# mrmod/h264decode

Hardware: AMD Instinct MI355X
Metric: 1080p Main CABAC frames/sec (higher is better)
Workload: dtype u8; 1 GPU; 1920x1080 Main CABAC IPPP GOP-30, 256 independent streams per GPU (32 distinct, each used 8 times), QP 28, 1 slice/frame, 1 ref; parallelism=streams sharded, no collective

## Files before the change

### h264decode_amd/csrc/k_entropy.hip

```cpp
#include <hip/hip_runtime.h>
#include "mi_kernels.h"

#ifndef MI_ENT_ISLICE_PRIO
#define MI_ENT_ISLICE_PRIO 0
#endif
#ifndef MI_ENT_MINWAVES
#define MI_ENT_MINWAVES 6
#endif
#ifndef MI_ENT_B
#define MI_ENT_B 0
#endif
#ifndef MI_ENT_FMO
#define MI_ENT_FMO MI_ENT_B
#endif
#ifndef MI_ENT_CABAC
#define MI_ENT_CABAC 0
#endif
#if MI_ENT_CABAC
#define ENT_CABAC(e) 1
#define IF_CAVLC(x) 0
#else
#define ENT_CABAC(e) ((e).cabac)
#define IF_CAVLC(x) (x)
#endif
// ... 26 lines not shown
    int8_t ipm[4];
    uint8_t nnz[8];
    int8_t ref[2][2];
    int16_t mv[NL][4][2];
    uint8_t mvd[NL][4][2];
};
#define TOP_DW (static_cast<int>(sizeof(TopInfo) / 4))
static_assert(sizeof(TopInfo) == (MI_ENT_B ? 72 : 48), "TopInfo layout");

struct Shared {
    uint8_t ctx[464];
#if !MI_ENT_CABAC
    uint8_t posmap[4][64];
#endif
    int16_t coef[MI_COEF_PER_MB];
    MbRec rec;
    TopInfo nb[4];
    int8_t ipm_c[32];
    uint8_t nnz_c[32];
    uint8_t nnzc_c[2][12];
    int8_t ref_c[NL][32];
    int8_t refi_c[NL][32];
    alignas(4) int16_t mv_c[NL][32][2];
    alignas(2) uint8_t mvd_c[NL][32][2];
    uint16_t parts[16];
    int8_t refs8[2][4];
    int8_t sub_type[4];
    uint8_t cur_cbf_dc, pad[3];
    int16_t ref_slot[NL][MI_MAX_REFS];
    uint32_t skip_tmpl[32];
    uint32_t role[64];
#if !MI_ENT_CABAC
    uint16_t vlc[MI_VLC_N];
#endif
    uint8_t coded[64];
#if MI_ENT_B
    uint32_t col[20];
    alignas(4) int16_t dmv[2][16][2];
    int8_t dref[2][4];
    int16_t dsf[MI_MAX_REFS];
#endif
};
#define GI(bx, by) (((by) + 1) * 6 + (bx) + 1)
enum { NB_LEFT = 0, NB_TL = 1, NB_TOP = 2 };

struct Ent {
    int lane;
    Shared *s;
    TopInfo *top;
    uint32_t pre_top;
// ... 498 lines not shown
        const int idx = st - 1, bx = (idx & 1) + 2 * ((idx >> 2) & 1), by = ((idx >> 1) & 1) + 2 * (idx >> 3);
        return static_cast<uint32_t>(GI(bx - 1, by)) | static_cast<uint32_t>(GI(bx, by - 1)) << 6 | static_cast<uint32_t>(GI(bx, by)) << 12 |
               static_cast<uint32_t>((by * 4 + bx) * 4) << 18 | 1u << 26;
    }
    if (st <= 18) {
        const uint32_t c = st - 17;
        return (51u + c) | (54u + c) << 6 | (57u + c) << 12 | (MI_COEF_CDC / 4 + c) << 18 | 2u << 26;
    }
    if (st <= 26) {
        const int j = st - 19, c = j >> 2, bx = j & 1, by = (j >> 1) & 1, g = 32 + 9 * c;
        return static_cast<uint32_t>(g + (by + 1) * 3 + bx) | static_cast<uint32_t>(g + by * 3 + bx + 1) << 6 | static_cast<uint32_t>(g + (by + 1) * 3 + bx + 1) << 12 |
               static_cast<uint32_t>(MI_COEF_CAC / 4 + j * 4) << 18 | 3u << 26;
    }
    return 0;
}
FI void parse_residual_cabac(Ent &e, int cbp_luma, int cbp_chroma, int t8x8) {
    Shared *s = e.s;
    const int i16 = e.cur_type == MBT_I16x16;
    int nl = LANE;
    OPAQUE(nl);
    const uint32_t cd = s->coded[nl];
    uint32_t vnz = (cd == 1 || (cd == 2 && MB_IS_INTRA(e.cur_type))) ? 1u : 0u;
    const uint32_t spread = (cbp_luma & 1) | (cbp_luma & 2) << 3 | (cbp_luma & 4) << 6 | (cbp_luma & 8) << 9;
    uint32_t steps = static_cast<uint32_t>(i16) | (spread * (t8x8 ? 1u : 15u)) << 1;
    if (cbp_chroma) steps |= 3u << 17;
    if (cbp_chroma & 2) steps |= 0xFFu << 19;
    const uint32_t cats = 0u | (t8x8 ? 5u : (i16 ? 1u : 2u)) << 4 | 3u << 8 | 4u << 12;
    while (steps) {
        const int step = __builtin_ctz(steps);
        steps &= steps - 1;
        const uint32_t d = RDL(e.v_step, step);
        const int cat = static_cast<int>((cats >> ((d >> 24) & 12u)) & 15);
        const int own = static_cast<int>((d >> 12) & 63);
        const int dst = cat == 5 ? (step - 1) * 16 : static_cast<int>((d >> 18) & 255) * 4;
        const int inc = static_cast<int>(RDL(vnz, d) + 2 * RDL(vnz, d >> 6));
        slide_window(e);
        if (cabac_residual(e, s->coef + dst, cat, inc)) {
            const uint64_t m = (cat == 5 ? 0xC3ull : 1ull) << own;
            asm("v_cndmask_b32_e64 %0, %0, 1, %1" : "+v"(vnz) : "s"(m));
        }
    }
    const uint64_t nzm = __builtin_amdgcn_ballot_w64(vnz != 0);
    const uint32_t lo = static_cast<uint32_t>(nzm);
    const uint32_t nzmask = ((lo >> GI(0, 0)) & 15) | ((lo >> GI(0, 1)) & 15) << 4 | ((lo >> GI(0, 2)) & 15) << 8 | ((lo >> GI(0, 3)) & 15) << 12;
    s->rec.nzmask = static_cast<uint16_t>(nzmask);
    s->cur_cbf_dc = static_cast<uint8_t>((nzm >> 56) & 7);
    int l = LANE;
    OPAQUE(l);
    const int bit = static_cast<int>(vnz);
    if (l < 30) {
        const int gx = l % 6 - 1, gy = l / 6 - 1;
        if (gx >= 0 && gx < 4 && gy >= 0) s->nnz_c[l] = static_cast<uint8_t>(bit);
    } else if (l >= 32 && l < 50) {
        const int i = l - 32, g = i % 9, gx = g % 3 - 1, gy = g / 3 - 1;
        if (gx >= 0 && gy >= 0) s->nnzc_c[i / 9][g] = static_cast<uint8_t>(bit);
    }
}

#if !MI_ENT_CABAC
FI void parse_residual_cavlc(Ent &e, int cbp_luma, int cbp_chroma, int t8x8) {
    Shared *s = e.s;
    const int i16 = e.cur_type == MBT_I16x16;
    int nzmask = 0, dc = 0;
    int nl = LANE;
    OPAQUE(nl);
    uint32_t vnn = nl < 30 ? s->nnz_c[nl] : ((nl >= 32 && nl < 56) ? (&s->nnzc_c[0][0])[nl - 32] : 0u);
    for (int step = 0; step < 27; step++) {
        int kind, bx = 0, by = 0, la = 0, lb = 0, own = 63, pmul = 1, padd = 0;
        int16_t *dst;
        if (step == 0) {
            if (!i16) continue;
            kind = 0;
            dst = s->coef + MI_COEF_I16DC;
            la = GI(-1, 0), lb = GI(0, -1);
        } else if (step <= 16) {
// ... 26 lines not shown
            la = 32 + 12 * c + (by + 1) * 3 + bx, lb = 32 + 12 * c + by * 3 + bx + 1, own = 32 + 12 * c + (by + 1) * 3 + bx + 1;
        }
        slide_window(e);
        const int nC = kind == 2 ? -1 : nc_of(static_cast<uint8_t>(RDL(vnn, la)), static_cast<uint8_t>(RDL(vnn, lb)));
        const int n = cavlc_residual(e, dst, kind, nC, pmul, padd);
        if (step == 0)
            dc |= n ? 1 : 0;
        else if (step <= 16) {
            vnn = nl == own ? static_cast<uint32_t>(n) : vnn;
            if (n) nzmask |= t8x8 ? (0x33 << ((by & 2) * 4 + (bx & 2))) : (1 << (by * 4 + bx));
        } else if (step <= 18)
            dc |= n ? 2 << (step - 17) : 0;
        else
            vnn = nl == own ? static_cast<uint32_t>(n) : vnn;
    }
    if (dc) s->cur_cbf_dc |= static_cast<uint8_t>(dc);
    s->rec.nzmask = static_cast<uint16_t>(nzmask);
    if (nl < 30) {
        const int gx = nl % 6 - 1, gy = nl / 6 - 1;
        if (gx >= 0 && gx < 4 && gy >= 0) s->nnz_c[nl] = static_cast<uint8_t>(vnn);
    } else if (nl >= 32 && nl < 56) {
        const int g = (nl - 32) % 12, gx = g % 3 - 1, gy = g / 3 - 1;
        if (g < 9 && gx >= 0 && gy >= 0) (&s->nnzc_c[0][0])[nl - 32] = static_cast<uint8_t>(vnn);
    }
}
#endif

FI int median3(int a, int b, int c) {
    int mn = a < b ? a : b, mx = a < b ? b : a;
    return c < mn ? mn : (c > mx ? mx : c);
}
FI void predict_mv(const Ent &e, const int L, int bx, int by, int w, int ref, int shape, int &px, int &py) {
    const Shared *s = e.s;
    int ia = GI(bx - 1, by), ib = GI(bx, by - 1), ic = GI(bx + w, by - 1);
    int ra = s->ref_c[L][ia], rb = s->ref_c[L][ib], rc = s->ref_c[L][ic];
    if (rc == -2) {
        ic = GI(bx - 1, by - 1);
        rc = s->ref_c[L][ic];
    }
// ... 56 lines not shown
        uint32_t off = NO_SRC, left = 0;
        if (gy < 0 && gx >= 0)
            off = NB_TOP * TB + static_cast<uint32_t>(offsetof(TopInfo, nnz)) + 4 + cpl * 2 + gx;
        else if (gx < 0 && gy >= 0)
            off = NB_LEFT * TB + static_cast<uint32_t>(offsetof(TopInfo, nnz)) + 4 + cpl * 2 + gy, left = 1;
        const uint32_t interior = gx >= 0 && gy >= 0;
        return off | interior << 12 | left << 14 | static_cast<uint32_t>(cpl * 12 + g) << 16;
    }
    if (l >= 50 && l < 56) {
        const uint32_t left = l < 53;
        return ((left ? NB_LEFT : NB_TOP) * TB + static_cast<uint32_t>(offsetof(TopInfo, cbf_dc))) | static_cast<uint32_t>((l - 50) % 3) << 9 | left << 14;
    }
    return NO_SRC;
}

FI void fill_caches(Ent &e) {
    Shared *s = e.s;
    const bool a_ok = (e.aw & 255) != 0, b_ok = (e.bw & 255) != 0;
    const int cip = e.cip;
    int l = LANE;
    OPAQUE(l);
    const uint32_t role = s->role[l], off = role & NO_SRC;
    const uint8_t *nbb = reinterpret_cast<const uint8_t *>(s->nb);
    int coded = 0;
    if (l < 30) {
        int8_t ipm = -2;
        uint8_t nnz = 0x80;
        const int k = static_cast<int>((role >> 9) & 3u);
        const bool has = off != NO_SRC && !((role >> 13) & 1u && e.mbx + 1 >= e.wmb);
        const TopInfo *n = reinterpret_cast<const TopInfo *>(nbb + (off != NO_SRC ? off : 0u));
        const bool n_ok = has && n->type != MBT_NONE;
        if (n_ok) {
            const int inter = MB_IS_INTER(n->type);
            if (!(cip && inter)) ipm = (n->type == MBT_I4x4 || n->type == MBT_I8x8) ? n->ipm[k] : static_cast<int8_t>(2);
            if ((role >> 11) & 1u) nnz = n->nnz[k];
        }
#pragma unroll
        for (int L = 0; L < NL; L++) {
            int8_t ref = -2, refi = -2;
            uint8_t mvdx = 0, mvdy = 0;
            int16_t mvx = 0, mvy = 0;
            if (n_ok) {
                if (MB_IS_INTER(n->type)) {
                    ref = refi = n->ref[L][k >> 1];
                    mvx = n->mv[L][k][0], mvy = n->mv[L][k][1];
                    mvdx = n->mvd[L][k][0], mvdy = n->mvd[L][k][1];
                    if (MI_ENT_B && ((n->dmask >> (k >> 1)) & 1)) refi = 0;
                } else
                    ref = refi = -1;
            }
            s->ref_c[L][l] = ref;
            s->refi_c[L][l] = refi;
            s->mv_c[L][l][0] = mvx, s->mv_c[L][l][1] = mvy;
            s->mvd_c[L][l][0] = mvdx, s->mvd_c[L][l][1] = mvdy;
        }
        if ((role >> 12) & 1u) {
            nnz = 0;
            ipm = -1;
        }
        coded = (nnz & 0x80) ? 2 : (nnz != 0);
        s->ipm_c[l] = ipm;
        e.v_ipm = ipm;
        s->nnz_c[l] = nnz;
    } else if (l >= 32 && l < 50) {
        const bool ok = off != NO_SRC && (((role >> 14) & 1u) ? a_ok : b_ok);
        const uint8_t v = ((role >> 12) & 1u) ? static_cast<uint8_t>(0) : (ok ? nbb[off != NO_SRC ? off : 0u] : static_cast<uint8_t>(0x80));
        coded = (v & 0x80) ? 2 : (v != 0);
        (&s->nnzc_c[0][0])[(role >> 16) & 31u] = v;
    } else if (l >= 50 && l < 56) {
        const bool ok = ((role >> 14) & 1u) ? a_ok : b_ok;
        coded = ok ? (nbb[off] >> ((role >> 9) & 3u)) & 1 : 2;
    } else if (l >= 56) {
        s->refs8[(l - 56) >> 2][l & 3] = -1;
        if (l < 60) s->sub_type[l - 56] = 0;
        if (l == 60) s->cur_cbf_dc = 0;
    }
    s->coded[l] = static_cast<uint8_t>(coded);
    LDS_SYNC();
}

#if MI_ENT_B
FI int min_positive(int a, int b) { return (a >= 0 && b >= 0) ? min(a, b) : max(a, b); }
FI int b_pair_modes(int k) { return static_cast<int>((0xFB7ED69A5ull >> (4 * k)) & 15); }
FI int b_sub_mode(int st) { return static_cast<int>((0x39FA5E4u >> (2 * st)) & 3); }
FI int b_sub_shape(int st) { return static_cast<int>((0x3F99900u >> (2 * st)) & 3); }
static_assert(((0x39FA5E4u >> 8) & 3) == 1 && ((0x39FA5E4u >> 24) & 3) == 3 && ((0x39FA5E4u >> 12) & 3) == 2 && ((0x3F99900u >> 8) & 3) == 1 && ((0x3F99900u >> 10) & 3) == 2,
              "Table 7-18 constants");

FI void direct_pred(Ent &e, int mask8, bool commit) {
    Shared *s = e.s;
    int l = LANE;
    OPAQUE(l);
    if (l < 20) s->col[l] = e.v_col;
// ... 171 lines not shown
        reinterpret_cast<uint32_t *>(e.top + e.mbx)[l] = nw;
        e.pre_top = top_load(e, e.mbx + 3, l);
    } else if (l >= 32) {
        const int k = l - 32;
        const uint32_t t = s->skip_tmpl[k];
        const uint32_t w = k == 0 ? (static_cast<uint32_t>(MBT_PSKIP) | e.qpw0) : (k == 1 ? e.qpw1 : ((k >= 12 && k < 28) ? mvw : t));
        const uint64_t mbi = e.mb_base + static_cast<uint64_t>(e.mby) * e.wmb + e.mbx;
        reinterpret_cast<uint32_t *>(e.mbrec + mbi)[k] = w;
    }
    LDS_SYNC();
}
#endif

FI void decode_mb(Ent &e, int skipped) {
    Shared *s = e.s;
    MbRec &r = s->rec;
    const int cabac = ENT_CABAC(e), islice = e.islice;
    int cbp_luma = 0, cbp_chroma = 0, t8x8 = 0, i16mode = 0, chroma_mode = 0, has_coef = 0;
    int type, raw = 0, nparts = 0;
    const Nb a{e.aw}, b{e.bw};
    r.nzmask = 0;
#if MI_ENT_B
    int no_sub8 = 1;
    e.direct8 = 0;
#endif
    if (skipped) {
#if MI_ENT_B
        type = MBT_BSKIP;
        e.cur_type = type;
        e.direct8 = 15;
        direct_pred(e, 15, true);
#else
        type = MBT_PSKIP;
        e.cur_type = type;
        int mvx = 0, mvy = 0;
        int ra = s->ref_c[0][GI(-1, 0)], rb = s->ref_c[0][GI(0, -1)];
        bool zero = ra == -2 || rb == -2 || (ra == 0 && s->mv_c[0][GI(-1, 0)][0] == 0 && s->mv_c[0][GI(-1, 0)][1] == 0) ||
                    (rb == 0 && s->mv_c[0][GI(0, -1)][0] == 0 && s->mv_c[0][GI(0, -1)][1] == 0);
        if (!zero) predict_mv(e, 0, 0, 0, 4, 0, 0, mvx, mvy);
        set_part(e, 0, 0, 0, 4, 4, 0, mvx, mvy, 0, 0);
        s->refs8[0][0] = s->refs8[0][1] = s->refs8[0][2] = s->refs8[0][3] = 0;
#endif
        e.prev_dqp_nz = 0;
    } else {
        MI_S(e, 3);
        int intra_prefix = 1;
        if (cabac) {
#if MI_ENT_B
            {
                intra_prefix = 0;
                const int inc = (a.ok() && a.type() != MBT_BSKIP && a.type() != MBT_BDIRECT) + (b.ok() && b.type() != MBT_BSKIP && b.type() != MBT_BDIRECT);
                if (!BIN_A(e, 27 + inc))
                    raw = 0;
                else if (!BIN_A(e, 27 + 3))
                    raw = 1 + BINI_A(e, 27 + 5);
                else {
                    int bits = BINI_A(e, 27 + 4) << 3;
                    bits |= BINI_A(e, 27 + 5) << 2;
                    bits |= BINI_A(e, 27 + 5) << 1;
// ... 57 lines not shown
        } else if (it == 25)
            type = MBT_IPCM;
        else {
            e.err = 20;
            type = MBT_I4x4;
        }
        e.cur_type = type;
        MI_S(e, 0);
        if (type == MBT_IPCM) {
            uint32_t pos = bitpos(e);
            if (cabac) pos -= static_cast<uint32_t>(RFL(e.avail));
            seek(e, (pos + 7) & ~7u);
            uint32_t *pcm = reinterpret_cast<uint32_t *>(s->coef);
            for (int i = 0; i < 96; i++) pcm[i] = (e.mono && i >= 64) ? 0x80808080u : __builtin_bswap32(get_bits(e, 32));
            if (cabac) cabac_start(e);
            for (int i = 0; i < 16; i++) {
                s->nnz_c[GI(i & 3, i >> 2)] = 16, s->ref_c[0][GI(i & 3, i >> 2)] = -1;
                if (MI_ENT_B) s->ref_c[NL - 1][GI(i & 3, i >> 2)] = -1;
            }
            for (int i = 0; i < 8; i++) s->nnzc_c[i >> 2][(((i >> 1) & 1) + 1) * 3 + (i & 1) + 1] = 16;
            s->cur_cbf_dc = 7;
            r.nzmask = 0xFFFF;
            cbp_luma = 15, cbp_chroma = 2;
            has_coef = 1;
            e.prev_dqp_nz = 0;
        } else {
            if (MB_IS_INTER(type)) {
#if MI_ENT_B
                if (type == MBT_BDIRECT) {
                    e.direct8 = 15;
                    direct_pred(e, 15, true);
                    no_sub8 = e.d8inf;
                } else {
                    int nref_parts;
                    if (raw <= 3) {
                        s->parts[0] = static_cast<uint16_t>(PART(0, 0, 4, 4, 0) | (raw << 11));
                        nparts = nref_parts = 1;
// ... 60 lines not shown
                        }
#pragma unroll
                    for (int L = 0; L < 2; L++)
                        for (int i = 0; i < nparts; i++) {
                            const int p = s->parts[i], md = p >> 11;
                            const int bx = p & 3, by = (p >> 2) & 3;
                            if (md == 0)
                                commit_direct(e, L, (by >> 1) * 2 + (bx >> 1));
                            else if ((md >> L) & 1)
                                read_mv(e, L, p);
                            else
                                set_part(e, L, bx, by, ((p >> 4) & 3) + 1, ((p >> 6) & 3) + 1, -1, 0, 0, 0, 0);
                        }
                }
#else
                int nref_parts;
                if (type == MBT_P16x16) {
                    s->parts[0] = PART(0, 0, 4, 4, 0);
                    nparts = nref_parts = 1;
                } else if (type == MBT_P16x8) {
                    s->parts[0] = PART(0, 0, 4, 2, 1), s->parts[1] = PART(0, 2, 4, 2, 2);
                    nparts = nref_parts = 2;
                } else if (type == MBT_P8x16) {
                    s->parts[0] = PART(0, 0, 2, 4, 3), s->parts[1] = PART(2, 0, 2, 4, 4);
                    nparts = nref_parts = 2;
                } else {
                    nref_parts = 4;
                    for (int i = 0; i < 4; i++) {
                        int st;
                        if (cabac)
// ... 14 lines not shown
                        bx = (i & 1) * 2, by = (i >> 1) * 2, w = 2, h = 2;
                    else {
                        const int p = s->parts[i];
                        bx = p & 3, by = (p >> 2) & 3, w = ((p >> 4) & 3) + 1, h = ((p >> 6) & 3) + 1;
                    }
                    read_ref_idx(e, 0, bx, by, w, h, raw != 4 ? e.nref : 1);
                }
                for (int i = 0; i < nparts; i++) read_mv(e, 0, s->parts[i]);
#endif
            } else {
                if (type == MBT_I4x4 && e.t8x8_mode) {
                    t8x8 = cabac ? BINI_T8(e, (a.ok() && a.t8x8()) + (b.ok() && b.t8x8())) : IF_CAVLC(static_cast<int>(get_bit(e)));
                    if (t8x8) type = MBT_I8x8, e.cur_type = type;
                }
                if (type == MBT_I4x4 || type == MBT_I8x8) {
                    const int n = type == MBT_I8x8 ? 4 : 16;
                    for (int i = 0; i < n; i++) {
                        int bx, by;
                        if (n == 4)
                            bx = (i & 1) * 2, by = (i >> 1) * 2;
                        else
                            bx = (i & 1) + 2 * ((i >> 2) & 1), by = ((i >> 1) & 1) + 2 * (i >> 3);
                        const int pa = static_cast<int>(RDL(e.v_ipm, GI(bx - 1, by))), pb = static_cast<int>(RDL(e.v_ipm, GI(bx, by - 1)));
                        const int pred = (pa < -1 || pb < -1) ? 2 : (pa < pb ? pa : pb);
                        int mode = pred;
                        if (cabac) {
                            if (!BIN_B(e, 68)) {
                                int rem = 0;
                                for (int k = 0; k < 3; k++) rem |= BINI_B(e, 69) << k;
                                mode = rem < pred ? rem : rem + 1;
// ... 9 lines not shown
                }
                if (e.mono)
                    chroma_mode = 0;
                else if (cabac) {
                    int inc = (a.ok() && MB_IS_INTRA(a.type()) && a.type() != MBT_IPCM && a.chroma_mode() != 0) +
                              (b.ok() && MB_IS_INTRA(b.type()) && b.type() != MBT_IPCM && b.chroma_mode() != 0);
                    chroma_mode = 0;
                    if (BIN_B(e, 64 + inc)) {
                        chroma_mode = 1;
                        while (chroma_mode < 3 && BIN_B(e, 67)) chroma_mode++;
                    }
                } else {
                    chroma_mode = IF_CAVLC(static_cast<int>(get_ue(e)));
                    if (chroma_mode > 3) e.err = 22, chroma_mode = 0;
                }
                if (LANE < 16) {
                    s->ref_c[0][GI(LANE & 3, LANE >> 2)] = -1;
                    if (MI_ENT_B) s->ref_c[NL - 1][GI(LANE & 3, LANE >> 2)] = -1;
                }
            }
            MI_S(e, MB_IS_INTER(type) ? 1 : 2);
            if (type != MBT_I16x16) {
                int cbp;
                if (cabac) {
                    const int cbp_a = a.ok() ? (a.type() == MBT_IPCM ? 0x2F : a.cbp()) : 0x0F;
                    const int cbp_b = b.ok() ? (b.type() == MBT_IPCM ? 0x2F : b.cbp()) : 0x0F;
                    cbp = 0;
                    for (int b8 = 0; b8 < 4; b8++) {
                        int ca = (b8 & 1) ? (cbp >> (b8 - 1)) & 1 : (cbp_a >> (b8 + 1)) & 1;
                        int cb = (b8 & 2) ? (cbp >> (b8 - 2)) & 1 : (cbp_b >> (b8 + 2)) & 1;
                        cbp |= BINI_B(e, 73 + (!ca) + 2 * (!cb)) << b8;
                    }
                    int ca = a.ok() && (a.type() == MBT_IPCM || (a.cbp() >> 4) != 0), cb = b.ok() && (b.type() == MBT_IPCM || (b.cbp() >> 4) != 0);
                    if (!e.mono && BIN_B(e, 77 + ca + 2 * cb)) {
// ... 26 lines not shown
                    while (BIN_A(e, 60 + ctx)) {
                        ctx = 2 + (ctx >> 1);
                        if (++val > 104) {
                            e.err = 2;
                            break;
                        }
                    }
                    dqp = (val & 1) ? (val + 1) >> 1 : -((val + 1) >> 1);
                } else
                    dqp = IF_CAVLC(get_se(e));
                if (dqp < -26 || dqp > 25) e.err = 24, dqp = 0;
                e.prev_dqp_nz = dqp != 0;
                if (dqp) set_qp(e, (e.qp + dqp + 52) % 52);
                MI_S(e, 2);
                MI_T(e, 1);
                MI_R0(e);
                if (cabac)
                    parse_residual_cabac(e, cbp_luma, cbp_chroma, t8x8);
                else
                    IF_CAVLC((parse_residual_cavlc(e, cbp_luma, cbp_chroma, t8x8), 0));
                MI_R(e, 3);
                MI_T(e, 2);
                has_coef = 1;
            } else
                e.prev_dqp_nz = 0;
        }
    }
    MI_T(e, 1);
    const int qp_store = type == MBT_IPCM ? 0 : e.qp;
    r.type = static_cast<uint8_t>(type);
    r.t8x8 = static_cast<uint8_t>(t8x8);
    r.qp = static_cast<uint8_t>(qp_store);
    r.qpc[0] = static_cast<uint8_t>(RDL(e.v_qpc, min(max(qp_store + e.cqp_off0, 0), 51)));
    r.qpc[1] = static_cast<uint8_t>(RDL(e.v_qpc, min(max(qp_store + e.cqp_off1, 0), 51)));
    r.cbp = static_cast<uint8_t>(cbp_luma | (cbp_chroma << 4));
    r.chroma_mode = static_cast<uint8_t>(chroma_mode);
    r.i16mode = static_cast<uint8_t>(i16mode);
    {
        const int cip = e.cip;
        int av = 0;
        if (MB_IS_INTRA(type)) {
            const int td = s->nb[NB_TL].type, tc = nb_ok(e, NB_TOP + 1) ? s->nb[NB_TOP + 1].type : MBT_NONE;
            if (a.ok() && !(cip && MB_IS_INTER(a.type()))) av |= MI_AV_LEFT;
            if (b.ok() && !(cip && MB_IS_INTER(b.type()))) av |= MI_AV_TOP;
            if (td != MBT_NONE && !(cip && MB_IS_INTER(td))) av |= MI_AV_TOPLEFT;
            if (tc != MBT_NONE && !(cip && MB_IS_INTER(tc))) av |= MI_AV_TOPRIGHT;
        }
        r.avail = static_cast<uint8_t>(av);
    }
    LDS_SYNC();
    int l = LANE;
    OPAQUE(l);
    const int inter = MB_IS_INTER(type);
    uint32_t cmask = 0, coff = 0;
    if (has_coef) {
        bool nz = false;
        if (l < MI_COEF_BLOCKS) {
            const uint4 a = reinterpret_cast<const uint4 *>(s->coef)[2 * l], b = reinterpret_cast<const uint4 *>(s->coef)[2 * l + 1];
            nz = (a.x | a.y | a.z | a.w | b.x | b.y | b.z | b.w) != 0;
        }
        cmask = static_cast<uint32_t>(__builtin_amdgcn_ballot_w64(nz));
        if (type == MBT_IPCM) cmask = 0xFFFu;
        const uint32_t n = static_cast<uint32_t>(__builtin_popcount(cmask));
        if (n && e.coef_cur + n > e.coef_end) {
            uint32_t base = 0;
            if (l == 0) base = atomicAdd(e.pool_head, static_cast<uint32_t>(MI_COEF_CHUNK));
            base = RFL(base);
            if (base + MI_COEF_CHUNK > e.pool_blocks) {
                e.err = 40;
                cmask = 0;
            } else
                e.coef_cur = base, e.coef_end = base + MI_COEF_CHUNK;
        }
        coff = e.coef_cur;
        e.coef_cur += static_cast<uint32_t>(__builtin_popcount(cmask));
    }
    if (l == 0) r.coef_off = coff, r.coef_mask = cmask;
    if (l < 16) {
        int g = GI(l & 3, l >> 2);
        int8_t v = s->ipm_c[g];
        if (inter) v = (MI_ENT_B && l < 4) ? s->refs8[NL - 1][l] : (l == 4 ? static_cast<int8_t>(raw) : ((l >= 5 && l < 9) ? s->sub_type[l - 5] : static_cast<int8_t>(0)));
        r.ipm[l] = v;
        r.mv[l][0] = inter ? s->mv_c[0][g][0] : static_cast<int16_t>(0);
        r.mv[l][1] = inter ? s->mv_c[0][g][1] : static_cast<int16_t>(0);
    } else if (l < 20) {
        int i = l - 16, ref = inter ? s->refs8[0][i] : -1;
        r.ref[i] = static_cast<int8_t>(ref);
        r.refslot[i] = ref >= 0 ? s->ref_slot[0][ref & (MI_MAX_REFS - 1)] : static_cast<int16_t>(-1);
    }
#if MI_ENT_B
    else if (l < 24) {
        const int i = l - 20, ref = inter ? s->refs8[1][i] : -1;
        r.refslot1[i] = ref >= 0 ? s->ref_slot[1][ref & (MI_MAX_REFS - 1)] : static_cast<int16_t>(-1);
    }
#endif
// ... 8 lines not shown
        dst->chroma_mode = static_cast<uint8_t>(chroma_mode);
        dst->cbf_dc = s->cur_cbf_dc;
        if (MI_ENT_FMO) dst->row = static_cast<uint16_t>(e.mby + 1);
#pragma unroll
        for (int L = 0; L < NL; L++) {
            dst->ref[L][0] = inter ? s->refs8[L][l == 0 ? 2 : 1] : static_cast<int8_t>(-1);
            dst->ref[L][1] = inter ? s->refs8[L][3] : static_cast<int8_t>(-1);
        }
#if MI_ENT_B
        dst->dmask = static_cast<uint8_t>(l == 0 ? (e.direct8 >> 2) & 3 : ((e.direct8 >> 1) & 1) | ((e.direct8 >> 2) & 2));
#endif
    } else if (l >= 8 && l < 16) {
        int k = l & 3, is_left = l >= 12;
        TopInfo *dst = &s->nb[is_left ? NB_LEFT : NB_TOP];
        int g = is_left ? GI(3, k) : GI(k, 3);
        dst->ipm[k] = s->ipm_c[g];
        dst->nnz[k] = s->nnz_c[g];
#pragma unroll
        for (int L = 0; L < NL; L++) {
            dst->mv[L][k][0] = s->mv_c[L][g][0], dst->mv[L][k][1] = s->mv_c[L][g][1];
            dst->mvd[L][k][0] = s->mvd_c[L][g][0], dst->mvd[L][k][1] = s->mvd_c[L][g][1];
        }
    } else if (l >= 16 && l < 24) {
        int i = l - 16, is_left = i >= 4, cpl = (i >> 1) & 1, k = i & 1;
        TopInfo *dst = &s->nb[is_left ? NB_LEFT : NB_TOP];
        dst->nnz[4 + cpl * 2 + k] = is_left ? s->nnzc_c[cpl][(k + 1) * 3 + 2] : s->nnzc_c[cpl][2 * 3 + k + 1];
    }
    LDS_SYNC();
    if (l < TOP_DW) {
        const uint32_t nw = reinterpret_cast<const uint32_t *>(tp)[l], w1 = reinterpret_cast<const uint32_t *>(&s->nb[NB_TOP + 1])[l];
        reinterpret_cast<uint32_t *>(e.top + e.mbx)[l] = nw;
        reinterpret_cast<uint32_t *>(&s->nb[NB_TOP])[l] = w1;
        reinterpret_cast<uint32_t *>(&s->nb[NB_TOP + 1])[l] = e.pre_top;
        e.pre_top = top_load(e, e.mbx + 3, l);
    }
    const uint64_t mbi = e.mb_base + static_cast<uint64_t>(e.mby) * e.wmb + e.mbx;
    if (l >= 32)
        reinterpret_cast<uint32_t *>(e.mbrec + mbi)[l - 32] = reinterpret_cast<const uint32_t *>(&r)[l - 32];
#if MI_ENT_B
    if (l < 16) reinterpret_cast<uint32_t *>(e.mbmv1 + mbi)[l] = inter ? *reinterpret_cast<const uint32_t *>(s->mv_c[1][GI(l & 3, l >> 2)]) : 0u;
#endif
    if (l < MI_COEF_BLOCKS && ((cmask >> l) & 1)) {
        uint4 *dst = reinterpret_cast<uint4 *>(e.coefs) + 2 * (static_cast<size_t>(coff) + __builtin_popcount(cmask & ((1u << l) - 1u)));
        dst[0] = reinterpret_cast<const uint4 *>(s->coef)[2 * l], dst[1] = reinterpret_cast<const uint4 *>(s->coef)[2 * l + 1];
        reinterpret_cast<uint4 *>(s->coef)[2 * l] = make_uint4(0, 0, 0, 0), reinterpret_cast<uint4 *>(s->coef)[2 * l + 1] = make_uint4(0, 0, 0, 0);
    }
    LDS_SYNC();
}

FI void fill_none(const Ent &e, int from, int to) {
    const int l = LANE;
    for (int a = from + (l >> 5); a < to; a += 2) reinterpret_cast<uint32_t *>(e.mbrec + e.mb_base + static_cast<uint64_t>(a))[l & 31] = 0u;
}

#if MI_ENT_B
extern "C" __global__ void __launch_bounds__(64) __attribute__((amdgpu_waves_per_eu(4, 8))) k_entropy_b(const SliceDesc *slices_, const PicDesc *pics, const uint8_t *bitstream, const DevTables *tab, MbRec *mbrec,
                                                           int16_t *coefs, uint32_t *pool_head, uint32_t pool_blocks, uint32_t *status_, uint32_t *toprows_, int wmb_max, uint32_t slice_base,
                                                           const BSliceExt *bexts, MbMv1 *mbmv1) {
#else
extern "C" __global__ void __launch_bounds__(64) __attribute__((amdgpu_waves_per_eu(MI_ENT_MINWAVES, 8))) MI_ENT_KERNEL(const SliceDesc *slices_, const PicDesc *pics, const uint8_t *bitstream, const DevTables *tab, MbRec *mbrec,
                                                           int16_t *coefs, uint32_t *pool_head, uint32_t pool_blocks, uint32_t *status_, uint32_t *toprows_, int wmb_max, uint32_t slice_base) {
#endif
// ... 72 lines not shown
    }
#endif
    {
        const int set = e.islice ? 0 : 1 + sd->cabac_init_idc;
        const uint8_t *src = tab->ctx_init[set][sd->slice_qp];
        e.ca = ctx_word(src[l]);
        e.cb = ctx_word(src[l < 61 ? 64 + l : 399 + (l - 61)]);
        e.wk = 0;
        e.wk_cat = -1, e.wk_c0 = 0, e.wk_home = 0, e.wk_valid = 0;
        for (int i = l; i < 464; i += 64) sh.ctx[i] = src[i];
    }
#if !MI_ENT_CABAC
    if (!pd->cabac)
        for (int i = l; i < MI_VLC_N / 2; i += 64) reinterpret_cast<uint32_t *>(sh.vlc)[i] = reinterpret_cast<const uint32_t *>(tab->vlc_c)[i];
#endif
    if (l < 32) reinterpret_cast<uint32_t *>(&sh.rec)[l] = 0;
    LDS_SYNC();
#if !MI_ENT_CABAC
    if (!pd->cabac) e.v_cat0 = l < 48 ? sh.vlc[MI_VLC_RUN + l] : 0u;
#endif
    if (l == 0) {
        sh.rec.dbf_idc = sd->dbf_idc;
        sh.rec.alpha_off = sd->alpha_off, sh.rec.beta_off = sd->beta_off;
        sh.rec.slice_in_pic = sd->slice_in_pic;
        sh.rec.slice_idx = slice_no;
        sh.rec.refslot1[0] = sh.rec.refslot1[1] = sh.rec.refslot1[2] = sh.rec.refslot1[3] = -1;
    }
    if (l < 32) {
        const uint32_t slot0 = static_cast<uint16_t>(sd->ref_slot[0]);
        sh.skip_tmpl[l] = l == 2 ? static_cast<uint32_t>(sd->dbf_idc) << 24
                                 : (l == 3 ? (static_cast<uint32_t>(static_cast<uint8_t>(sd->alpha_off)) | static_cast<uint32_t>(static_cast<uint8_t>(sd->beta_off)) << 8 |
                                              static_cast<uint32_t>(sd->slice_in_pic) << 16)
                                           : ((l == 9 || l == 10) ? (slot0 | slot0 << 16) : (l == 11 ? slice_no : (l >= 30 ? 0xFFFFFFFFu : 0u))));
    }
    for (int i = l; i < MI_COEF_PER_MB / 2; i += 64) reinterpret_cast<uint32_t *>(sh.coef)[i] = 0;
    sh.role[l] = build_role(l);
    for (int i = l; i < e.wmb * TOP_DW; i += 64) reinterpret_cast<uint32_t *>(e.top)[i] = 0;
    if (l < TOP_DW) reinterpret_cast<uint32_t *>(&sh.nb[NB_LEFT])[l] = 0, reinterpret_cast<uint32_t *>(&sh.nb[NB_TL])[l] = 0;
    if (l < 2 * TOP_DW) reinterpret_cast<uint32_t *>(&sh.nb[NB_TOP])[l] = 0;
    LDS_SYNC();
    {
        uint32_t pos = RFL(sd->data_bit_off);
        if (ENT_CABAC(e)) pos = (pos + 7) & ~7u;
        e.wbase = 0x80000000u;
        seek(e, pos);
        if (ENT_CABAC(e)) cabac_start(e);
    }
    const int total = min(e.wmb * e.hmb, RFL(static_cast<int>(sd->end_mb)));
#if !MI_ENT_CABAC
// ... 54 lines not shown
                    if (pending > 0) skip_state = 1;
                }
                if (skip_state == 1) {
                    skipped = 1;
                    pending--;
                }
            }
#endif
        }
#if !MI_ENT_B
        if (skipped) {
            MI_T(e, 1);
            pskip_fast(e);
        } else
#endif
        {
            MI_T(e, 1);
            fill_caches(e);
            MI_T(e, 0);
            decode_mb(e, skipped);
        }
        MI_T(e, 3);
        if (e.err) break;
        n_mbs++;
        if (ENT_CABAC(e))
            more = !cabac_terminate(e);
#if !MI_ENT_CABAC
        else if (skipped) {
            if (pending == 0) {
                more = bitpos(e) < stop_bit;
                skip_state = 2;
            }
        } else {
            more = bitpos(e) < stop_bit;
            skip_state = 0;
        }
// ... 37 lines not shown
```

Before: 29940 frames/s.

## Split neighbour cache fill into lazy per-need phases and write MB records directly

Replaces the monolithic fill_caches with fill_always, fill_motion, fill_ipm and fill_resid. In non-B builds each is invoked only when the macroblock type needs it (motion for inter, ipm for NxN intra, residual context before residual parsing). The coded-flag context is passed in registers instead of through LDS, and the nzmask/cbf_dc results are returned instead of stored. For non-B builds the LDS MbRec staging is dropped: record words and neighbour TopInfo words are assembled per lane and written straight to global memory. This cuts LDS traffic and barriers per macroblock on the serial entropy path, at the cost of a large, duplicated store path that is error-prone for intra/inter edge cases.

```diff
diff --git a/h264decode_amd/csrc/k_entropy.hip b/h264decode_amd/csrc/k_entropy.hip
--- a/h264decode_amd/csrc/k_entropy.hip
+++ b/h264decode_amd/csrc/k_entropy.hip
@@ -64,7 +64,9 @@
     uint8_t posmap[4][64];
 #endif
     int16_t coef[MI_COEF_PER_MB];
+#if MI_ENT_B
     MbRec rec;
+#endif
     TopInfo nb[4];
     int8_t ipm_c[32];
     uint8_t nnz_c[32];
@@ -74,16 +76,17 @@
     alignas(4) int16_t mv_c[NL][32][2];
     alignas(2) uint8_t mvd_c[NL][32][2];
     uint16_t parts[16];
-    int8_t refs8[2][4];
-    int8_t sub_type[4];
+    alignas(4) int8_t refs8[2][4];
+    alignas(4) int8_t sub_type[4];
+#if MI_ENT_B
     uint8_t cur_cbf_dc, pad[3];
+#endif
     int16_t ref_slot[NL][MI_MAX_REFS];
     uint32_t skip_tmpl[32];
     uint32_t role[64];
 #if !MI_ENT_CABAC
     uint16_t vlc[MI_VLC_N];
 #endif
-    uint8_t coded[64];
 #if MI_ENT_B
     uint32_t col[20];
     alignas(4) int16_t dmv[2][16][2];
@@ -612,12 +615,9 @@
     }
     return 0;
 }
-FI void parse_residual_cabac(Ent &e, int cbp_luma, int cbp_chroma, int t8x8) {
+FI uint32_t parse_residual_cabac(Ent &e, const uint32_t cd, int cbp_luma, int cbp_chroma, int t8x8) {
     Shared *s = e.s;
     const int i16 = e.cur_type == MBT_I16x16;
-    int nl = LANE;
-    OPAQUE(nl);
-    const uint32_t cd = s->coded[nl];
     uint32_t vnz = (cd == 1 || (cd == 2 && MB_IS_INTRA(e.cur_type))) ? 1u : 0u;
     const uint32_t spread = (cbp_luma & 1) | (cbp_luma & 2) << 3 | (cbp_luma & 4) << 6 | (cbp_luma & 8) << 9;
     uint32_t steps = static_cast<uint32_t>(i16) | (spread * (t8x8 ? 1u : 15u)) << 1;
@@ -641,8 +641,7 @@
     const uint64_t nzm = __builtin_amdgcn_ballot_w64(vnz != 0);
     const uint32_t lo = static_cast<uint32_t>(nzm);
     const uint32_t nzmask = ((lo >> GI(0, 0)) & 15) | ((lo >> GI(0, 1)) & 15) << 4 | ((lo >> GI(0, 2)) & 15) << 8 | ((lo >> GI(0, 3)) & 15) << 12;
-    s->rec.nzmask = static_cast<uint16_t>(nzmask);
-    s->cur_cbf_dc = static_cast<uint8_t>((nzm >> 56) & 7);
+    const uint32_t cbf_dc = static_cast<uint32_t>(nzm >> 56) & 7u;
     int l = LANE;
     OPAQUE(l);
     const int bit = static_cast<int>(vnz);
@@ -653,10 +652,11 @@
         const int i = l - 32, g = i % 9, gx = g % 3 - 1, gy = g / 3 - 1;
         if (gx >= 0 && gy >= 0) s->nnzc_c[i / 9][g] = static_cast<uint8_t>(bit);
     }
+    return nzmask | cbf_dc << 16;
 }
 
 #if !MI_ENT_CABAC
-FI void parse_residual_cavlc(Ent &e, int cbp_luma, int cbp_chroma, int t8x8) {
+FI uint32_t parse_residual_cavlc(Ent &e, int cbp_luma, int cbp_chroma, int t8x8) {
     Shared *s = e.s;
     const int i16 = e.cur_type == MBT_I16x16;
     int nzmask = 0, dc = 0;
@@ -713,8 +713,6 @@
         else
             vnn = nl == own ? static_cast<uint32_t>(n) : vnn;
     }
-    if (dc) s->cur_cbf_dc |= static_cast<uint8_t>(dc);
-    s->rec.nzmask = static_cast<uint16_t>(nzmask);
     if (nl < 30) {
         const int gx = nl % 6 - 1, gy = nl / 6 - 1;
         if (gx >= 0 && gx < 4 && gy >= 0) s->nnz_c[nl] = static_cast<uint8_t>(vnn);
@@ -722,6 +720,7 @@
         const int g = (nl - 32) % 12, gx = g % 3 - 1, gy = g / 3 - 1;
         if (g < 9 && gx >= 0 && gy >= 0) (&s->nnzc_c[0][0])[nl - 32] = static_cast<uint8_t>(vnn);
     }
+    return static_cast<uint32_t>(nzmask) | static_cast<uint32_t>(dc) << 16;
 }
 #endif
 
@@ -808,33 +807,45 @@
     return NO_SRC;
 }
 
-FI void fill_caches(Ent &e) {
+FI void fill_always(Ent &e) {
     Shared *s = e.s;
-    const bool a_ok = (e.aw & 255) != 0, b_ok = (e.bw & 255) != 0;
-    const int cip = e.cip;
     int l = LANE;
     OPAQUE(l);
-    const uint32_t role = s->role[l], off = role & NO_SRC;
-    const uint8_t *nbb = reinterpret_cast<const uint8_t *>(s->nb);
-    int coded = 0;
+    if (l >= 56) {
+        s->refs8[(l - 56) >> 2][l & 3] = -1;
+        if (l < 60) s->sub_type[l - 56] = 0;
+#if MI_ENT_B
+        if (l == 60) s->cur_cbf_dc = 0;
+#endif
+    }
+    LDS_SYNC();
+}
+struct NbSrc {
+    const TopInfo *n;
+    uint32_t role;
+    int k;
+    bool ok;
+};
+FI NbSrc nb_src(const Ent &e, int l) {
+    const uint32_t role = e.s->role[l], off = role & NO_SRC;
+    const bool has = off != NO_SRC && !((role >> 13) & 1u && e.mbx + 1 >= e.wmb);
+    const TopInfo *n = reinterpret_cast<const TopInfo *>(reinterpret_cast<const uint8_t *>(e.s->nb) + (off != NO_SRC ? off : 0u));
+    return NbSrc{n, role, static_cast<int>((role >> 9) & 3u), has && n->type != MBT_NONE};
+}
+FI void fill_motion(Ent &e) {
+    Shared *s = e.s;
+    int l = LANE;
+    OPAQUE(l);
     if (l < 30) {
-        int8_t ipm = -2;
-        uint8_t nnz = 0x80;
-        const int k = static_cast<int>((role >> 9) & 3u);
-        const bool has = off != NO_SRC && !((role >> 13) & 1u && e.mbx + 1 >= e.wmb);
-        const TopInfo *n = reinterpret_cast<const TopInfo *>(nbb + (off != NO_SRC ? off : 0u));
-        const bool n_ok = has && n->type != MBT_NONE;
-        if (n_ok) {
-            const int inter = MB_IS_INTER(n->type);
-            if (!(cip && inter)) ipm = (n->type == MBT_I4x4 || n->type == MBT_I8x8) ? n->ipm[k] : static_cast<int8_t>(2);
-            if ((role >> 11) & 1u) nnz = n->nnz[k];
-        }
+        const NbSrc c = nb_src(e, l);
+        const TopInfo *n = c.n;
+        const int k = c.k;
 #pragma unroll
         for (int L = 0; L < NL; L++) {
             int8_t ref = -2, refi = -2;
             uint8_t mvdx = 0, mvdy = 0;
             int16_t mvx = 0, mvy = 0;
-            if (n_ok) {
+            if (c.ok) {
                 if (MB_IS_INTER(n->type)) {
                     ref = refi = n->ref[L][k >> 1];
                     mvx = n->mv[L][k][0], mvy = n->mv[L][k][1];
@@ -848,29 +859,48 @@
             s->mv_c[L][l][0] = mvx, s->mv_c[L][l][1] = mvy;
             s->mvd_c[L][l][0] = mvdx, s->mvd_c[L][l][1] = mvdy;
         }
-        if ((role >> 12) & 1u) {
-            nnz = 0;
-            ipm = -1;
-        }
+    }
+    LDS_SYNC();
+}
+FI void fill_ipm(Ent &e) {
+    int l = LANE;
+    OPAQUE(l);
+    if (l < 30) {
+        const NbSrc c = nb_src(e, l);
+        int ipm = -2;
+        if (c.ok && !(e.cip && MB_IS_INTER(c.n->type))) ipm = (c.n->type == MBT_I4x4 || c.n->type == MBT_I8x8) ? c.n->ipm[c.k] : 2;
+        if ((c.role >> 12) & 1u) ipm = -1;
+        e.v_ipm = ipm;
+    }
+}
+FI uint32_t fill_resid(Ent &e) {
+    Shared *s = e.s;
+    const bool a_ok = (e.aw & 255) != 0, b_ok = (e.bw & 255) != 0;
+    const bool counts = !ENT_CABAC(e);
+    int l = LANE;
+    OPAQUE(l);
+    const uint8_t *nbb = reinterpret_cast<const uint8_t *>(s->nb);
+    int coded = 0;
+    if (l < 30) {
+        const NbSrc c = nb_src(e, l);
+        uint8_t nnz = 0x80;
+        if (c.ok && ((c.role >> 11) & 1u)) nnz = c.n->nnz[c.k];
+        if ((c.role >> 12) & 1u) nnz = 0;
         coded = (nnz & 0x80) ? 2 : (nnz != 0);
-        s->ipm_c[l] = ipm;
-        e.v_ipm = ipm;
-        s->nnz_c[l] = nnz;
+        if (counts) s->nnz_c[l] = nnz;
     } else if (l >= 32 && l < 50) {
+        const uint32_t role = s->role[l], off = role & NO_SRC;
         const bool ok = off != NO_SRC && (((role >> 14) & 1u) ? a_ok : b_ok);
         const uint8_t v = ((role >> 12) & 1u) ? static_cast<uint8_t>(0) : (ok ? nbb[off != NO_SRC ? off : 0u] : static_cast<uint8_t>(0x80));
         coded = (v & 0x80) ? 2 : (v != 0);
-        (&s->nnzc_c[0][0])[(role >> 16) & 31u] = v;
+        if (counts) (&s->nnzc_c[0][0])[(role >> 16) & 31u] = v;
     } else if (l >= 50 && l < 56) {
+        const uint32_t role = s->role[l], off = role & NO_SRC;
         const bool ok = ((role >> 14) & 1u) ? a_ok : b_ok;
         coded = ok ? (nbb[off] >> ((role >> 9) & 3u)) & 1 : 2;
-    } else if (l >= 56) {
-        s->refs8[(l - 56) >> 2][l & 3] = -1;
-        if (l < 60) s->sub_type[l - 56] = 0;
-        if (l == 60) s->cur_cbf_dc = 0;
-    }
-    s->coded[l] = static_cast<uint8_t>(coded);
-    LDS_SYNC();
+    }
+    if (counts) LDS_SYNC();
+    return static_cast<uint32_t>(coded);
 }
 
 #if MI_ENT_B
@@ -1072,35 +1102,31 @@
 
 FI void decode_mb(Ent &e, int skipped) {
     Shared *s = e.s;
-    MbRec &r = s->rec;
     const int cabac = ENT_CABAC(e), islice = e.islice;
     int cbp_luma = 0, cbp_chroma = 0, t8x8 = 0, i16mode = 0, chroma_mode = 0, has_coef = 0;
     int type, raw = 0, nparts = 0;
+    uint32_t nz_dc = 0;
     const Nb a{e.aw}, b{e.bw};
-    r.nzmask = 0;
-#if MI_ENT_B
+    MI_T(e, 1);
+    fill_always(e);
+#if MI_ENT_B
+    fill_motion(e);
+    fill_ipm(e);
+    const uint32_t cd = fill_resid(e);
     int no_sub8 = 1;
     e.direct8 = 0;
 #endif
+    MI_T(e, 0);
+#if MI_ENT_B
     if (skipped) {
-#if MI_ENT_B
         type = MBT_BSKIP;
         e.cur_type = type;
         e.direct8 = 15;
         direct_pred(e, 15, true);
-#else
-        type = MBT_PSKIP;
-        e.cur_type = type;
-        int mvx = 0, mvy = 0;
-        int ra = s->ref_c[0][GI(-1, 0)], rb = s->ref_c[0][GI(0, -1)];
-        bool zero = ra == -2 || rb == -2 || (ra == 0 && s->mv_c[0][GI(-1, 0)][0] == 0 && s->mv_c[0][GI(-1, 0)][1] == 0) ||
-                    (rb == 0 && s->mv_c[0][GI(0, -1)][0] == 0 && s->mv_c[0][GI(0, -1)][1] == 0);
-        if (!zero) predict_mv(e, 0, 0, 0, 4, 0, 0, mvx, mvy);
-        set_part(e, 0, 0, 0, 4, 4, 0, mvx, mvy, 0, 0);
-        s->refs8[0][0] = s->refs8[0][1] = s->refs8[0][2] = s->refs8[0][3] = 0;
-#endif
         e.prev_dqp_nz = 0;
-    } else {
+    } else
+#endif
+    {
         MI_S(e, 3);
         int intra_prefix = 1;
         if (cabac) {
@@ -1188,13 +1214,9 @@
             uint32_t *pcm = reinterpret_cast<uint32_t *>(s->coef);
             for (int i = 0; i < 96; i++) pcm[i] = (e.mono && i >= 64) ? 0x80808080u : __builtin_bswap32(get_bits(e, 32));
             if (cabac) cabac_start(e);
-            for (int i = 0; i < 16; i++) {
-                s->nnz_c[GI(i & 3, i >> 2)] = 16, s->ref_c[0][GI(i & 3, i >> 2)] = -1;
-                if (MI_ENT_B) s->ref_c[NL - 1][GI(i & 3, i >> 2)] = -1;
-            }
+            for (int i = 0; i < 16; i++) s->nnz_c[GI(i & 3, i >> 2)] = 16;
             for (int i = 0; i < 8; i++) s->nnzc_c[i >> 2][(((i >> 1) & 1) + 1) * 3 + (i & 1) + 1] = 16;
-            s->cur_cbf_dc = 7;
-            r.nzmask = 0xFFFF;
+            nz_dc = 0xFFFFu | 7u << 16;
             cbp_luma = 15, cbp_chroma = 2;
             has_coef = 1;
             e.prev_dqp_nz = 0;
@@ -1285,6 +1307,9 @@
                         }
                 }
 #else
+                MI_T(e, 1);
+                fill_motion(e);
+                MI_T(e, 0);
                 int nref_parts;
                 if (type == MBT_P16x16) {
                     s->parts[0] = PART(0, 0, 4, 4, 0);
@@ -1329,6 +1354,11 @@
                     if (t8x8) type = MBT_I8x8, e.cur_type = type;
                 }
                 if (type == MBT_I4x4 || type == MBT_I8x8) {
+#if !MI_ENT_B
+                    MI_T(e, 1);
+                    fill_ipm(e);
+                    MI_T(e, 0);
+#endif
                     const int n = type == MBT_I8x8 ? 4 : 16;
                     for (int i = 0; i < n; i++) {
                         int bx, by;
@@ -1368,10 +1398,6 @@
                     chroma_mode = IF_CAVLC(static_cast<int>(get_ue(e)));
                     if (chroma_mode > 3) e.err = 22, chroma_mode = 0;
                 }
-                if (LANE < 16) {
-                    s->ref_c[0][GI(LANE & 3, LANE >> 2)] = -1;
-                    if (MI_ENT_B) s->ref_c[NL - 1][GI(LANE & 3, LANE >> 2)] = -1;
-                }
             }
             MI_S(e, MB_IS_INTER(type) ? 1 : 2);
             if (type != MBT_I16x16) {
@@ -1428,11 +1454,15 @@
                 if (dqp) set_qp(e, (e.qp + dqp + 52) % 52);
                 MI_S(e, 2);
                 MI_T(e, 1);
+#if !MI_ENT_B
+                const uint32_t cd = fill_resid(e);
+                MI_T(e, 0);
+#endif
                 MI_R0(e);
                 if (cabac)
-                    parse_residual_cabac(e, cbp_luma, cbp_chroma, t8x8);
+                    nz_dc = parse_residual_cabac(e, cd, cbp_luma, cbp_chroma, t8x8);
                 else
-                    IF_CAVLC((parse_residual_cavlc(e, cbp_luma, cbp_chroma, t8x8), 0));
+                    nz_dc = IF_CAVLC(parse_residual_cavlc(e, cbp_luma, cbp_chroma, t8x8));
                 MI_R(e, 3);
                 MI_T(e, 2);
                 has_coef = 1;
@@ -1441,6 +1471,10 @@
         }
     }
     MI_T(e, 1);
+#if MI_ENT_B
+    MbRec &r = s->rec;
+    r.nzmask = static_cast<uint16_t>(nz_dc);
+    s->cur_cbf_dc = static_cast<uint8_t>(nz_dc >> 16);
     const int qp_store = type == MBT_IPCM ? 0 : e.qp;
     r.type = static_cast<uint8_t>(type);
     r.t8x8 = static_cast<uint8_t>(t8x8);
@@ -1466,6 +1500,7 @@
     int l = LANE;
     OPAQUE(l);
     const int inter = MB_IS_INTER(type);
+    const bool nxn = type == MBT_I4x4 || type == MBT_I8x8;
     uint32_t cmask = 0, coff = 0;
     if (has_coef) {
         bool nz = false;
@@ -1492,7 +1527,7 @@
     if (l == 0) r.coef_off = coff, r.coef_mask = cmask;
     if (l < 16) {
         int g = GI(l & 3, l >> 2);
-        int8_t v = s->ipm_c[g];
+        int8_t v = nxn ? s->ipm_c[g] : static_cast<int8_t>(-1);
         if (inter) v = (MI_ENT_B && l < 4) ? s->refs8[NL - 1][l] : (l == 4 ? static_cast<int8_t>(raw) : ((l >= 5 && l < 9) ? s->sub_type[l - 5] : static_cast<int8_t>(0)));
         r.ipm[l] = v;
         r.mv[l][0] = inter ? s->mv_c[0][g][0] : static_cast<int16_t>(0);
@@ -1531,17 +1566,17 @@
         int k = l & 3, is_left = l >= 12;
         TopInfo *dst = &s->nb[is_left ? NB_LEFT : NB_TOP];
         int g = is_left ? GI(3, k) : GI(k, 3);
-        dst->ipm[k] = s->ipm_c[g];
-        dst->nnz[k] = s->nnz_c[g];
+        dst->ipm[k] = nxn ? s->ipm_c[g] : static_cast<int8_t>(-1);
+        dst->nnz[k] = has_coef ? s->nnz_c[g] : static_cast<uint8_t>(0);
 #pragma unroll
         for (int L = 0; L < NL; L++) {
-            dst->mv[L][k][0] = s->mv_c[L][g][0], dst->mv[L][k][1] = s->mv_c[L][g][1];
-            dst->mvd[L][k][0] = s->mvd_c[L][g][0], dst->mvd[L][k][1] = s->mvd_c[L][g][1];
+            *reinterpret_cast<uint32_t *>(dst->mv[L][k]) = inter ? *reinterpret_cast<const uint32_t *>(s->mv_c[L][g]) : 0u;
+            *reinterpret_cast<uint16_t *>(dst->mvd[L][k]) = inter ? *reinterpret_cast<const uint16_t *>(s->mvd_c[L][g]) : static_cast<uint16_t>(0);
         }
     } else if (l >= 16 && l < 24) {
         int i = l - 16, is_left = i >= 4, cpl = (i >> 1) & 1, k = i & 1;
         TopInfo *dst = &s->nb[is_left ? NB_LEFT : NB_TOP];
-        dst->nnz[4 + cpl * 2 + k] = is_left ? s->nnzc_c[cpl][(k + 1) * 3 + 2] : s->nnzc_c[cpl][2 * 3 + k + 1];
+        dst->nnz[4 + cpl * 2 + k] = !has_coef ? static_cast<uint8_t>(0) : (is_left ? s->nnzc_c[cpl][(k + 1) * 3 + 2] : s->nnzc_c[cpl][2 * 3 + k + 1]);
     }
     LDS_SYNC();
     if (l < TOP_DW) {
@@ -1563,6 +1598,120 @@
         reinterpret_cast<uint4 *>(s->coef)[2 * l] = make_uint4(0, 0, 0, 0), reinterpret_cast<uint4 *>(s->coef)[2 * l + 1] = make_uint4(0, 0, 0, 0);
     }
     LDS_SYNC();
+#else
+    const int inter = MB_IS_INTER(type);
+    const bool nxn = type == MBT_I4x4 || type == MBT_I8x8;
+    const uint32_t cbp = static_cast<uint32_t>(cbp_luma | (cbp_chroma << 4));
+    uint32_t rw0, rw1;
+    if (type == MBT_IPCM) {
+        rw0 = static_cast<uint32_t>(type) | RDL(e.v_qpc, min(max(e.cqp_off0, 0), 51)) << 24;
+        rw1 = RDL(e.v_qpc, min(max(e.cqp_off1, 0), 51)) & 255u;
+    } else
+        rw0 = static_cast<uint32_t>(type) | static_cast<uint32_t>(t8x8) << 8 | e.qpw0, rw1 = e.qpw1;
+    rw1 |= cbp << 8 | static_cast<uint32_t>(chroma_mode) << 16 | static_cast<uint32_t>(i16mode) << 24;
+    uint32_t rw2 = nz_dc & 0xFFFFu;
+    if (MB_IS_INTRA(type)) {
+        const int cip = e.cip;
+        const int td = s->nb[NB_TL].type, tc = nb_ok(e, NB_TOP + 1) ? s->nb[NB_TOP + 1].type : MBT_NONE;
+        uint32_t av = 0;
+        if (a.ok() && !(cip && MB_IS_INTER(a.type()))) av |= MI_AV_LEFT;
+        if (b.ok() && !(cip && MB_IS_INTER(b.type()))) av |= MI_AV_TOP;
+        if (td != MBT_NONE && !(cip && MB_IS_INTER(td))) av |= MI_AV_TOPLEFT;
+        if (tc != MBT_NONE && !(cip && MB_IS_INTER(tc))) av |= MI_AV_TOPRIGHT;
+        rw2 |= av << 16;
+    }
+    const uint32_t ew0 = static_cast<uint32_t>(type) | static_cast<uint32_t>(t8x8) << 8 | cbp << 16 | static_cast<uint32_t>(chroma_mode) << 24;
+    const uint32_t ew1 = (nz_dc >> 16) | (MI_ENT_FMO ? static_cast<uint32_t>(e.mby + 1) << 16 : 0u);
+    LDS_SYNC();
+    int l = LANE;
+    OPAQUE(l);
+    uint32_t cmask = 0, coff = 0;
+    if (has_coef) {
+        bool nz = false;
+        if (l < MI_COEF_BLOCKS) {
+            const uint4 a = reinterpret_cast<const uint4 *>(s->coef)[2 * l], b = reinterpret_cast<const uint4 *>(s->coef)[2 * l + 1];
+            nz = (a.x | a.y | a.z | a.w | b.x | b.y | b.z | b.w) != 0;
+        }
+        cmask = static_cast<uint32_t>(__builtin_amdgcn_ballot_w64(nz));
+        if (type == MBT_IPCM) cmask = 0xFFFu;
+        const uint32_t n = static_cast<uint32_t>(__builtin_popcount(cmask));
+        if (n && e.coef_cur + n > e.coef_end) {
+            uint32_t base = 0;
+            if (l == 0) base = atomicAdd(e.pool_head, static_cast<uint32_t>(MI_COEF_CHUNK));
+            base = RFL(base);
+            if (base + MI_COEF_CHUNK > e.pool_blocks) {
+                e.err = 40;
+                cmask = 0;
+            } else
+                e.coef_cur = base, e.coef_end = base + MI_COEF_CHUNK;
+        }
+        coff = e.coef_cur;
+        e.coef_cur += static_cast<uint32_t>(__builtin_popcount(cmask));
+    }
+    static_assert(offsetof(Shared, nnz_c) == offsetof(Shared, ipm_c) + 32 && offsetof(Shared, nnzc_c) == offsetof(Shared, ipm_c) + 64, "byte grids are consecutive");
+    const uint8_t *grid = reinterpret_cast<const uint8_t *>(s->ipm_c);
+    if (l < 32) {
+        const int d = l & 15, left = l >> 4;
+        const int g0 = left ? GI(3, 0) : GI(0, 3), gs = left ? 6 : 1;
+        uint32_t nw = d == 0 ? ew0 : (d == 1 ? ew1 : (d == 2 ? 0xFFFFFFFFu : (d == 5 ? 0x0000FFFFu : 0u)));
+        if (nxn || has_coef) {
+            const int s1 = d == 4 ? (left ? 3 : 1) : gs, s2 = d == 4 ? 12 : 2 * gs;
+            const int base = d == 4 ? 64 + (left ? 5 : 7) : (d == 3 ? 32 + g0 : g0);
+            const uint32_t gw = grid[base] | static_cast<uint32_t>(grid[base + s1]) << 8 | static_cast<uint32_t>(grid[base + s2]) << 16 | static_cast<uint32_t>(grid[base + s1 + s2]) << 24;
+            nw = (d == 2 ? nxn : ((d == 3 || d == 4) && has_coef)) ? gw : nw;
+        }
+        if (inter) {
+            const uint32_t r8 = *reinterpret_cast<const uint32_t *>(s->refs8[0]);
+            const uint32_t rw = left ? (((r8 >> 8) & 255u) | ((r8 >> 16) & 0xFF00u)) : (r8 >> 16);
+            const uint32_t mw = *reinterpret_cast<const uint32_t *>(s->mv_c[0][g0 + ((d - 6) & 3) * gs]);
+            const int g = g0 + 2 * (d & 1) * gs;
+            const uint32_t dw = *reinterpret_cast<const uint16_t *>(s->mvd_c[0][g]) | static_cast<uint32_t>(*reinterpret_cast<const uint16_t *>(s->mvd_c[0][g + gs])) << 16;
+            nw = d == 5 ? rw : ((d >= 6 && d < 10) ? mw : (d >= 10 ? dw : nw));
+        }
+        if (d < TOP_DW) {
+            if (left)
+                reinterpret_cast<uint32_t *>(&s->nb[NB_LEFT])[d] = nw;
+            else {
+                uint32_t *tl = reinterpret_cast<uint32_t *>(&s->nb[NB_TL]), *tp = reinterpret_cast<uint32_t *>(&s->nb[NB_TOP]), *tr = reinterpret_cast<uint32_t *>(&s->nb[NB_TOP + 1]);
+                const uint32_t old_top = tp[d], w1 = tr[d];
+                tl[d] = old_top;
+                tp[d] = w1;
+                tr[d] = e.pre_top;
+                reinterpret_cast<uint32_t *>(e.top + e.mbx)[d] = nw;
+                e.pre_top = top_load(e, e.mbx + 3, d);
+            }
+        }
+    } else {
+        const int k = l - 32;
+        const uint32_t t = s->skip_tmpl[k];
+        uint32_t w = k == 0 ? rw0 : (k == 1 ? rw1 : (k == 2 ? (t | rw2) : (k == 28 ? coff : (k == 29 ? cmask : t))));
+        if (inter) {
+            const uint32_t st = *reinterpret_cast<const uint32_t *>(s->sub_type), r8 = *reinterpret_cast<const uint32_t *>(s->refs8[0]);
+            const int h = 16 * ((k + 1) & 1);
+            const int r0 = static_cast<int8_t>((r8 >> h) & 255u), r1 = static_cast<int8_t>((r8 >> (h + 8)) & 255u);
+            const uint32_t s0 = r0 >= 0 ? static_cast<uint16_t>(s->ref_slot[0][r0 & (MI_MAX_REFS - 1)]) : 0xFFFFu;
+            const uint32_t s1 = r1 >= 0 ? static_cast<uint16_t>(s->ref_slot[0][r1 & (MI_MAX_REFS - 1)]) : 0xFFFFu;
+            const int i = (k - 12) & 15;
+            const uint32_t mw = *reinterpret_cast<const uint32_t *>(s->mv_c[0][GI(i & 3, i >> 2)]);
+            w = k == 5 ? ((static_cast<uint32_t>(raw) & 255u) | st << 8) : (k == 6 ? st >> 24 : (k == 8 ? r8 : ((k == 9 || k == 10) ? (s0 | s1 << 16) : ((k >= 12 && k < 28) ? mw : w))));
+        } else {
+            uint32_t iw = 0xFFFFFFFFu;
+            if (nxn) {
+                const int g = GI(0, k & 3);
+                iw = grid[g] | static_cast<uint32_t>(grid[g + 1]) << 8 | static_cast<uint32_t>(grid[g + 2]) << 16 | static_cast<uint32_t>(grid[g + 3]) << 24;
+            }
+            w = (k >= 4 && k < 8) ? iw : ((k >= 8 && k < 11) ? 0xFFFFFFFFu : w);
+        }
+        const uint64_t mbi = e.mb_base + static_cast<uint64_t>(e.mby) * e.wmb + e.mbx;
+        reinterpret_cast<uint32_t *>(e.mbrec + mbi)[k] = w;
+    }
+    if (l < MI_COEF_BLOCKS && ((cmask >> l) & 1)) {
+        uint4 *dst = reinterpret_cast<uint4 *>(e.coefs) + 2 * (static_cast<size_t>(coff) + __builtin_popcount(cmask & ((1u << l) - 1u)));
+        dst[0] = reinterpret_cast<const uint4 *>(s->coef)[2 * l], dst[1] = reinterpret_cast<const uint4 *>(s->coef)[2 * l + 1];
+        reinterpret_cast<uint4 *>(s->coef)[2 * l] = make_uint4(0, 0, 0, 0), reinterpret_cast<uint4 *>(s->coef)[2 * l + 1] = make_uint4(0, 0, 0, 0);
+    }
+    LDS_SYNC();
+#endif
 }
 
 FI void fill_none(const Ent &e, int from, int to) {
@@ -1665,18 +1814,21 @@
     if (!pd->cabac)
         for (int i = l; i < MI_VLC_N / 2; i += 64) reinterpret_cast<uint32_t *>(sh.vlc)[i] = reinterpret_cast<const uint32_t *>(tab->vlc_c)[i];
 #endif
+#if MI_ENT_B
     if (l < 32) reinterpret_cast<uint32_t *>(&sh.rec)[l] = 0;
+#endif
     LDS_SYNC();
 #if !MI_ENT_CABAC
     if (!pd->cabac) e.v_cat0 = l < 48 ? sh.vlc[MI_VLC_RUN + l] : 0u;
 #endif
+#if MI_ENT_B
     if (l == 0) {
         sh.rec.dbf_idc = sd->dbf_idc;
         sh.rec.alpha_off = sd->alpha_off, sh.rec.beta_off = sd->beta_off;
         sh.rec.slice_in_pic = sd->slice_in_pic;
         sh.rec.slice_idx = slice_no;
-        sh.rec.refslot1[0] = sh.rec.refslot1[1] = sh.rec.refslot1[2] = sh.rec.refslot1[3] = -1;
-    }
+    }
+#else
     if (l < 32) {
         const uint32_t slot0 = static_cast<uint16_t>(sd->ref_slot[0]);
         sh.skip_tmpl[l] = l == 2 ? static_cast<uint32_t>(sd->dbf_idc) << 24
@@ -1684,6 +1836,7 @@
                                               static_cast<uint32_t>(sd->slice_in_pic) << 16)
                                            : ((l == 9 || l == 10) ? (slot0 | slot0 << 16) : (l == 11 ? slice_no : (l >= 30 ? 0xFFFFFFFFu : 0u))));
     }
+#endif
     for (int i = l; i < MI_COEF_PER_MB / 2; i += 64) reinterpret_cast<uint32_t *>(sh.coef)[i] = 0;
     sh.role[l] = build_role(l);
     for (int i = l; i < e.wmb * TOP_DW; i += 64) reinterpret_cast<uint32_t *>(e.top)[i] = 0;
@@ -1768,12 +1921,7 @@
             pskip_fast(e);
         } else
 #endif
-        {
-            MI_T(e, 1);
-            fill_caches(e);
-            MI_T(e, 0);
             decode_mb(e, skipped);
-        }
         MI_T(e, 3);
         if (e.err) break;
         n_mbs++;
```

Result: no change. 29650 frames/s (-1.0%).
